# sahaRatul/sela

Hardware: AMD Instinct MI355X
Metric: Msamples/s encode+decode, 16-bit stereo 44.1kHz, 1/2/4/8 GPU; bit-exact vs CPU (higher is better)
Workload: dtype f64+int64

## Files before the change

### sela_amd/csrc/sela_device.h

```cpp
#ifndef SELA_DEVICE_H_
#define SELA_DEVICE_H_

#include <hip/hip_runtime.h>
#include <stdint.h>

#define SELA_TABLE_QUAL static __device__ const
#include "sela_format.h"
#include "sela_hip.h"
#include "sela_hip_debug.h"

namespace sela {

constexpr int kWave = 64;
constexpr int kBlock = SELA_BLOCK;
constexpr int kPerLane = kBlock / kWave;
constexpr int kMaxOrder = SELA_MAX_LPC_ORDER;
constexpr int kCoefWordsCap = 32;
constexpr int kResWordsCap = 2208;
constexpr int kSlotWords = kCoefWordsCap + kResWordsCap;
constexpr int kGroupFrames = 8;

struct BlockMeta {
    uint8_t order;
    uint8_t coef_k;
// ... 134 lines not shown
__device__ __forceinline__ uint32_t zigzag32(int32_t x)
{
    const uint32_t t = (uint32_t)x << 1;
    return x < 0 ? (0u - t - 1u) : t;
}
__device__ __forceinline__ uint32_t words_for_bits(uint64_t bits)
{
    return (uint32_t)ceilf((float)bits / 32.0f);
}

__device__ __forceinline__ double dequant(int i, int32_t q, uint32_t& flags)
{
    int idx = q + 64;
    if (idx < 0 || idx > 127) {
        flags |= SELA_HIP_FLAG_Q_RANGE;
        idx = idx < 0 ? 0 : 127;
    }
    return i == 0 ? SELA_DEQUANT_FIRST[idx] : (i == 1 ? SELA_DEQUANT_SECOND[idx] : SELA_DEQUANT_HIGHER[idx]);
}

__device__ __forceinline__ int64_t q35_trunc(double v, uint32_t& flags)
{
    const double scaled = 34359738368.0 * v;
    if (!(scaled > -9223372036854775808.0 && scaled < 9223372036854775808.0)) {
        flags |= SELA_HIP_FLAG_COEF_OVERFLOW;
        return INT64_MIN;
    }
    return (int64_t)scaled;
}

__device__ __forceinline__ double read_lane(double v, int src_lane )
{
    const uint64_t x = __builtin_bit_cast(uint64_t, v);
    const uint32_t lo = (uint32_t)__builtin_amdgcn_readlane((int)(uint32_t)x, src_lane);
    const uint32_t hi = (uint32_t)__builtin_amdgcn_readlane((int)(uint32_t)(x >> 32), src_lane);
    return __builtin_bit_cast(double, ((uint64_t)hi << 32) | lo);
}
__device__ __forceinline__ double wave_shr1_zero(double v)
{
    const uint64_t x = __builtin_bit_cast(uint64_t, v);
    const uint32_t lo = (uint32_t)__builtin_amdgcn_mov_dpp((int)(uint32_t)x, 0x138 , 0xf, 0xf, true);
    const uint32_t hi = (uint32_t)__builtin_amdgcn_mov_dpp((int)(uint32_t)(x >> 32), 0x138, 0xf, 0xf, true);
    return __builtin_bit_cast(double, ((uint64_t)hi << 32) | lo);
}
__device__ __forceinline__ double wave_shr1(double fill, double v)
{
    const uint64_t f = __builtin_bit_cast(uint64_t, fill), x = __builtin_bit_cast(uint64_t, v);
    const uint32_t lo = (uint32_t)__builtin_amdgcn_update_dpp((int)(uint32_t)f, (int)(uint32_t)x, 0x138 , 0xf, 0xf, false);
    const uint32_t hi = (uint32_t)__builtin_amdgcn_update_dpp((int)(uint32_t)(f >> 32), (int)(uint32_t)(x >> 32), 0x138, 0xf, 0xf, false);
    return __builtin_bit_cast(double, ((uint64_t)hi << 32) | lo);
}

__device__ inline void step_up_regs(double k_lo, double k_hi, int64_t* a, int order, int lane, uint32_t& flags)
{
    double t_lo = lane == 0 ? 1.0 : 0.0, r_lo = lane == 1 ? 1.0 : 0.0;
    double t_hi = 0.0, r_hi = 0.0;
    const int n_lo = order < 62 ? order : 62;
    for (int i = 0; i < n_lo; i++) {
        const double ki = read_lane(k_lo, i);
        const double tn = t_lo + ki * r_lo;
        const double rn = r_lo + ki * t_lo;
        t_lo = tn;
        r_lo = wave_shr1_zero(rn);
    }
    for (int i = 62; i < order; i++) {
        const double ki = i < 64 ? read_lane(k_lo, i) : read_lane(k_hi, i - 64);
        const double tn_lo = t_lo + ki * r_lo, rn_lo = r_lo + ki * t_lo;
        const double tn_hi = t_hi + ki * r_hi, rn_hi = r_hi + ki * t_hi;
        t_lo = tn_lo;
        t_hi = tn_hi;
        const double carry = read_lane(rn_lo, 63);
        r_lo = wave_shr1_zero(rn_lo);
        r_hi = wave_shr1(carry, rn_hi);
    }
    if (lane == 0)
        a[0] = 0;
    else if (lane <= order)
        a[lane] = q35_trunc(-t_lo, flags);
    if (lane + 64 <= order)
        a[lane + 64] = q35_trunc(-t_hi, flags);
    wave_sync();
}

__device__ inline void step_up(const double* kd, int64_t* a, int order, int lane, uint32_t& flags)
{
    const double k_lo = lane < order ? kd[lane] : 0.0;
    const double k_hi = lane + 64 < order ? kd[lane + 64] : 0.0;
    step_up_regs(k_lo, k_hi, a, order, lane, flags);
}

__device__ __forceinline__ void step_up_from_q(uint32_t order, int32_t q_lo, int32_t q_hi, int64_t* a, int lane, uint32_t& flags)
{
    int table_lane = lane;
    asm volatile("" : "+v"(table_lane));
    const double k_lo = (uint32_t)lane < order ? (order <= 1 ? 0.0 : dequant(table_lane, q_lo, flags)) : 0.0;
    const double k_hi = (uint32_t)lane + 64 < order ? dequant(64, q_hi, flags) : 0.0;
    step_up_regs(k_lo, k_hi, a, (int)order, lane, flags);
}

constexpr int kResidencyDecode = 0, kResidencyVerify = 1, kResidencySlots = 2;
uint32_t resident_frames(const void* kernel, int n_waves, size_t lds, int slot = kResidencyDecode);
uint32_t vec_shift_from_for(uint32_t n_frames, int n_waves, uint32_t resident);
int decode_waves(uint32_t channels);

}
#endif
```

### sela_amd/csrc/sela_encode.hip

```cpp
#include <algorithm>
#include <atomic>
#include <random>
#include <vector>

#include "sela_device.h"

namespace sela {

constexpr int kPadC = 64;
constexpr int kHalfEntries = kBlock / 4;
constexpr int kParityLen = kPadC + kHalfEntries + 64;
constexpr int kLastT0 = (kHalfEntries + 64) / 32 - 1;
constexpr int kFirstT1 = (kHalfEntries - kPadC) / 32;
constexpr int kRingHalf = 64;
constexpr int kRingLen = 2 * kRingHalf + 64;
constexpr int kRingsPerXcd = 512;
constexpr int kXcds = 8;
constexpr int kPadS = 128;
constexpr int kSBufWords = (kPadS + kBlock) / 32 * 33;
constexpr int kSmallBase = 8992;
constexpr int kBigBytes = kSmallBase + 3008;
static_assert(kResWordsCap * 4 <= kSmallBase, "packed residue words must fit the dead sample buffer");
static_assert(kSBufWords * 4 <= kSmallBase && kSmallBase % 16 == 0, "sample buffer must end below the analysis arrays");
static_assert(kBigBytes >= 2 * kParityLen * 8, "the FP64 parity arrays must fit");

struct SmallArrays {
    double ac[104];
    double k[104];
    int64_t a[104];
    int32_t q[128];
};
static_assert(sizeof(SmallArrays) + kSmallBase <= kBigBytes, "analysis arrays overflow the LDS plan");

__device__ __forceinline__ void or_bits(uint32_t* buf, uint32_t pos, uint32_t v, uint32_t nbits)
{
    const uint32_t w = pos >> 5, sh = pos & 31;
    atomicOr(&buf[w], v << sh);
    if (sh + nbits > 32)
        atomicOr(&buf[w + 1], v >> (32 - sh));
}

__device__ __forceinline__ void or_bits_both(uint32_t* buf, uint32_t pos, uint32_t v)
{
    const uint64_t wide = (uint64_t)v << (pos & 31);
    uint32_t* const w = buf + (pos >> 5);
    atomicOr(w, (uint32_t)wide);
    atomicOr(w + 1, (uint32_t)(wide >> 32));
}

__device__ __attribute__((noinline)) uint32_t put_long_codeword(uint32_t* buf, uint32_t pos, uint32_t u, uint32_t k);

__device__ __forceinline__ uint32_t put_codeword(uint32_t* buf, uint32_t pos, uint32_t u, uint32_t k)
{
    uint32_t ones = u >> k;
    const uint32_t rem = k ? (__brev(u << (32 - k))) : 0u;
    while (ones >= 32) {
        or_bits(buf, pos, 0xFFFFFFFFu, 32);
        pos += 32;
        ones -= 32;
    }
    if (ones + 1 + k <= 32) {
        or_bits(buf, pos, ((1u << ones) - 1u) | (rem << (ones + 1)), ones + 1 + k);
        return pos + ones + 1 + k;
    }
    or_bits(buf, pos, (1u << ones) - 1u, ones + 1);
    pos += ones + 1;
    if (k) {
        or_bits(buf, pos, rem, k);
        pos += k;
    }
    return pos;
}

__device__ __attribute__((noinline)) uint32_t put_long_codeword(uint32_t* buf, uint32_t pos, uint32_t u, uint32_t k)
{
    return put_codeword(buf, pos, u, k);
}

template <int V>
__device__ __forceinline__ uint64_t rice_shifted_sum(const uint32_t (&u)[V], uint32_t k, bool small, uint32_t& lane_part)
{
    if (small) {
        uint32_t part = 0;
#pragma unroll
        for (int t = 0; t < V; t++)
            part += u[t] >> k;
        asm volatile("" : "+v"(part));
        lane_part = part;
        return wave_sum_small(part);
    }
    uint64_t part = 0;
#pragma unroll
    for (int t = 0; t < V; t++)
        part += u[t] >> k;
    lane_part = (uint32_t)part;
    return wave_sum_40(part);
}

template <int V>
__device__ __forceinline__ void rice_plan(const uint32_t (&u)[V], uint32_t n, uint32_t& best_k, uint64_t& best_bits, uint32_t& lane_or, uint32_t& lane_quotients)
{
    constexpr uint32_t kLast = SELA_MAX_RICE_PARAM - 1;
    lane_or = 0;
#pragma unroll
    for (int t = 0; t < V; t++)
        lane_or |= u[t];
    const bool small = !__any((lane_or >> 20) != 0);
    uint32_t p0, pa, pb, pc;
    const uint64_t t0 = rice_shifted_sum<V>(u, 0, small, p0);
    const uint64_t mean = n ? t0 / n : 0;
    uint32_t k = mean ? 63u - (uint32_t)__clzll(mean) : 0u;
    k = k > kLast - 1 ? kLast - 1 : k;
    uint64_t ta = t0;
    pa = p0;
    if (k)
        ta = rice_shifted_sum<V>(u, k, small, pa);
    uint64_t tb = rice_shifted_sum<V>(u, k + 1, small, pb);
    if (ta - tb <= n) {
        while (k > 0) {
            uint64_t tc = t0;
            pc = p0;
            if (k != 1)
                tc = rice_shifted_sum<V>(u, k - 1, small, pc);
            if (tc - ta > n)
                break;
            k--;
            tb = ta, pb = pa;
            ta = tc, pa = pc;
        }
    } else {
        for (;;) {
            k++;
            ta = tb, pa = pb;
            if (k == kLast)
                break;
            tb = rice_shifted_sum<V>(u, k + 1, small, pb);
            if (ta - tb <= n)
                break;
        }
    }
    best_k = k;
    best_bits = ta + (uint64_t)n * (1 + k);
    lane_quotients = pa;
}

__device__ __forceinline__ double scale_sample(int32_t s)
{
    constexpr double c1 = 0x1.00020004p-15, c2 = 0x1.0002000400080p-60;
    static_assert(c1 == 1.0 / 32768 + 1.0 / (1 << 30) + 1.0 / (1ll << 45) && SELA_SAMPLE_SCALE == 32767.0, "the constants are those of a division by 32767");
    const double x = (double)s;
    const double q = x * c1;
    return __builtin_fma(x, c2, q);
}

template <int kN>
__device__ __forceinline__ void unpack_stereo(uint32_t sig, const uint32_t (&w)[kN], int32_t (&raw)[kN])
{
    if (sig == 0) {
#pragma unroll
        for (int i = 0; i < kN; i++)
            raw[i] = (int32_t)(int16_t)(w[i] & 0xFFFFu);
    } else if (sig == 1) {
#pragma unroll
        for (int i = 0; i < kN; i++)
            raw[i] = (int32_t)w[i] >> 16;
    } else {
#pragma unroll
        for (int i = 0; i < kN; i++)
            raw[i] = (int32_t)(int16_t)(w[i] & 0xFFFFu) - ((int32_t)w[i] >> 16);
    }
}

__device__ __forceinline__ uint32_t stereo_pick(uint32_t sig) { return sig == 0 ? 0x00000001u : sig == 1 ? 0x00010000u : 0xFFFF0001u; }
__device__ __forceinline__ int32_t unpack_stereo_picked(uint32_t pick, uint32_t w)
{
    int32_t s;
    asm("v_dot2_i32_i16 %0, %1, %2, 0" : "=v"(s) : "v"(w), "s"(pick));
    return s;
}

typedef double f64x2 __attribute__((ext_vector_type(2)));
struct MeanFetch {
    f64x2 e0, e1, e2, e3, o0, o1, o2, o3;
};
#define SELA_MEAN_STR2(x) #x
#define SELA_MEAN_STR(x) SELA_MEAN_STR2(x)
#define SELA_MEAN_ISSUE(F, addr, OFF, sum)                                                    \
    asm volatile("ds_read_b128 %0, %9 offset:" #OFF "+0\n\t"                                    \
                 "ds_read_b128 %4, %9 offset:" #OFF "+5120\n\t"                                 \
                 "ds_read_b128 %1, %9 offset:" #OFF "+16\n\t"                                   \
// ... 2163 lines not shown
```

### sela_amd/csrc/sela_encode_tail.inc

```

    SELA_STAMP(5);
#ifndef SELA_TAIL_HAVE_Q
    int order;
    {
        const unsigned long long b_lo = __ballot(fabs(k_lo) > SELA_ORDER_THRESHOLD);
        const unsigned long long b_hi = __ballot(lane < 36 && fabs(k_hi) > SELA_ORDER_THRESHOLD);
        order = b_hi ? 128 - __clzll(b_hi) : (b_lo ? 64 - __clzll(b_lo) : 1);
    }
#endif

    {
#ifndef SELA_TAIL_HAVE_Q
        const double sqrt2 = SELA_SQRT2;
        double v_lo;
        if (lane == 0)
            v_lo = floor(64 * (-1 + (sqrt2 * sqrt(k_lo + 1))));
        else if (lane == 1)
            v_lo = floor(64 * (-1 + (sqrt2 * sqrt(-k_lo + 1))));
        else
            v_lo = floor(64 * k_lo);
        const double v_hi = floor(64 * k_hi);
        const int32_t q_lo = isnan(v_lo) ? 0 : (int32_t)v_lo;
        const int32_t q_hi = isnan(v_hi) ? 0 : (int32_t)v_hi;
#endif
// ... 89 lines not shown
                const int32_t rt = (int32_t)((uint32_t)mine_s[t] - pred_u[t]);
                wide |= (rt >= (1 << 30)) || (rt < -(1 << 30));
            }
        } else {
            double* const c_first = reinterpret_cast<double*>(sm->a);
            double* const c_second = single ? c_first : sm->k;
            for (int j = 1 + lane; j <= order; j += 64) {
                const int64_t aj = sm->a[j];
                const int64_t top = aj >> 20;
                const double lo = (double)(uint32_t)((uint64_t)aj & 0xFFFFFu);
                const double hi = (double)(int32_t)(top >> 16) * 65536.0 + (double)(uint32_t)((uint64_t)top & 0xFFFFu);
                if (single) {
                    c_first[j] = hi * 1048576.0 + lo;
                } else {
                    c_first[j] = lo;
                    c_second[j] = hi;
                }
            }
            wave_sync();
            double win_f[kPerLane], acc_f[kPerLane];
            double half = (double)((int64_t)1 << (SELA_Q_SHIFT - 1));
            asm volatile("" : "+s"(half));
#pragma unroll
            for (int t = 0; t < kPerLane; t++)
                acc_f[t] = half;
            if (single) {
#pragma unroll
                for (int t = 0; t < kPerLane; t++)
                    win_f[t] = (double)mine_s[t];
#pragma unroll 1
                for (int j0 = 0; j0 < order; j0 += 32)
                    fir_taps_f64<0>(j0, order, fir_group_window(sT, lane, j0), fir_group_coefs(c_first, j0), win_f, acc_f);
#pragma unroll
                for (int t = 0; t < kPerLane; t++) {
                    if constexpr (kMode == 4)
                        pred_u[t] = (uint32_t)((int32_t)__builtin_ceil(acc_f[t] * (1.0 / (double)((int64_t)1 << SELA_Q_SHIFT))) - 1);
                    else
                        pred_u[t] = (uint32_t)(int32_t)__builtin_floor(acc_f[t] * (1.0 / (double)((int64_t)1 << SELA_Q_SHIFT)));
                }
            } else {
#pragma unroll 1
                for (int pass = 0; pass < 2; pass++) {
                    const double* const coef = pass ? c_second : c_first;
#pragma unroll
                    for (int t = 0; t < kPerLane; t++)
                        win_f[t] = (double)mine_s[t];
#pragma unroll 1
                    for (int j0 = 0; j0 < order; j0 += 32)
                        fir_taps_f64<0>(j0, order, fir_group_window(sT, lane, j0), fir_group_coefs(coef, j0), win_f, acc_f);
                    const double down = pass ? 1.0 / (double)((int64_t)1 << (SELA_Q_SHIFT - 20)) : 1.0 / 1048576.0;
#pragma unroll
                    for (int t = 0; t < kPerLane; t++) {
                        if constexpr (kMode == 4)
                            acc_f[t] = __builtin_ceil(acc_f[t] * down);
                        else
                            acc_f[t] = __builtin_floor(acc_f[t] * down);
                    }
                }
#pragma unroll
                for (int t = 0; t < kPerLane; t++) {
                    if constexpr (kMode == 4)
                        pred_u[t] = (uint32_t)((int32_t)acc_f[t] - 1);
                    else
                        pred_u[t] = (uint32_t)(int32_t)acc_f[t];
                }
            }
        }
#pragma unroll
        for (int t = 0; t < kPerLane; t++) {
            const int32_t rt = (int32_t)((uint32_t)mine_s[t] - pred_u[t]);
            ru[t] = zigzag32(rt);
#ifdef SELA_TAIL_TRACE_RESIDUES
            if (kTrace && (SELA_TAIL_TRACE_RESIDUES))
                (SELA_TAIL_TRACE_RESIDUES)[(size_t)block_id * kBlock + 32 * lane + t] = rt;
#endif
        }
    }
    wave_sync();

    SELA_STAMP(8);
    uint32_t cu[2];
    cu[0] = 2 * lane < order ? zigzag32(sm->q[2 * lane]) : 0u;
    cu[1] = 2 * lane + 1 < order ? zigzag32(sm->q[2 * lane + 1]) : 0u;
    uint32_t coef_k, coef_or, coef_quotients;
    uint64_t coef_bits;
    rice_plan<2>(cu, (uint32_t)order, coef_k, coef_bits, coef_or, coef_quotients);
    const uint32_t coef_words = words_for_bits(coef_bits);

    if (__any(wide))
        flags |= SELA_HIP_FLAG_RICE_RANGE;
    uint32_t res_k, res_or, res_quotients;
    uint64_t res_bits;
    rice_plan<kPerLane>(ru, (uint32_t)kBlock, res_k, res_bits, res_or, res_quotients);
    uint32_t res_words = words_for_bits(res_bits);
    if (res_words > (uint32_t)kResWordsCap || coef_words > (uint32_t)kCoefWordsCap) {
        flags |= SELA_HIP_FLAG_WORDS_CAP;
        res_words = 0;
    }

    const bool paired = sizes_pub != nullptr && channels == 2 && sig >= 1;
    const uint32_t my_words = coef_words + res_words;
    if (paired && lane == 0)
        store_through(sizes_pub + block_id, sizes_tag | (uint64_t)my_words);

    SELA_STAMP(9);
    if (lane < kCoefWordsCap)
        cw_buf[lane] = 0;
    wave_sync();
    if (!(flags & SELA_HIP_FLAG_WORDS_CAP)) {
        const uint32_t n0 = 2 * lane < order ? (cu[0] >> coef_k) + 1 + coef_k : 0u;
        const uint32_t n1 = 2 * lane + 1 < order ? (cu[1] >> coef_k) + 1 + coef_k : 0u;
        uint32_t pos = wave_exclusive_scan(n0 + n1, lane);
        if (n0)
            pos = put_codeword(cw_buf, pos, cu[0], coef_k);
        if (n1)
            pos = put_codeword(cw_buf, pos, cu[1], coef_k);
    }

    uint64_t other = 0;
    if (paired)
        other = load_through(sizes_pub + (sig == 1 ? block_id + 1 : block_id - 1));

    SELA_STAMP(10);
    uint32_t* const out_words = reinterpret_cast<uint32_t*>(big);
    for (uint32_t w = lane; w < res_words; w += 64)
        out_words[w] = 0;
    const uint32_t lane_bits = res_quotients + (uint32_t)kPerLane * (1 + res_k);
    wave_sync();
    if (res_words) {
        uint32_t pos = wave_exclusive_scan(lane_bits, lane);
#pragma unroll
        for (int t = 0; t < kPerLane; t++) {
            const uint32_t u = ru[t], ones = u >> res_k, len = ones + 1 + res_k;
            if (len <= 32) {
                const uint32_t rem = __builtin_amdgcn_ubfe(__brev(u), 32 - res_k, res_k);
                or_bits_both(out_words, pos, ((1u << ones) - 1u) | (rem << ((ones + 1) & 31)));
                pos += len;
            } else {
                pos = put_long_codeword(out_words, pos, u, res_k);
            }
        }
    }
    wave_sync();

    SELA_STAMP(11);
    uint32_t* slot = slots + (size_t)block_id * kSlotWords;
    bool loser = false;
    if (paired) {
        const uint32_t other_words = (uint32_t)other & 0xFFFu;
        loser = (other & ~(uint64_t)0xFFF) == sizes_tag && (sig == 1 ? other_words < my_words : !(my_words < other_words));
        loser = __builtin_amdgcn_readfirstlane((int)loser) != 0;
    }
    if (loser) {
    } else if (kFused) {
        uint64_t* const slot2 = reinterpret_cast<uint64_t*>(slot);
        if (lane < kCoefWordsCap / 2)
            store_through(slot2 + lane, (uint64_t)cw_buf[2 * lane] | ((uint64_t)cw_buf[2 * lane + 1] << 32));
        const uint64_t* const out2 = reinterpret_cast<const uint64_t*>(out_words);
        for (uint32_t w2 = lane; w2 < (res_words + 1) / 2; w2 += 64)
            store_through(slot2 + kCoefWordsCap / 2 + w2, out2[w2]);
    } else {
        if (lane < (int)coef_words && lane < kCoefWordsCap)
            slot[lane] = cw_buf[lane];
        for (uint32_t w = lane; w < res_words; w += 64)
            slot[kCoefWordsCap + w] = out_words[w];
    }
    const uint32_t all_flags = wave_or(flags);
    if (lane == 0) {
        BlockMeta bm;
        bm.order = (uint8_t)order;
        bm.coef_k = (uint8_t)coef_k;
        bm.res_k = (uint8_t)res_k;
        bm.flags = (uint8_t)(all_flags | form_bits);
        bm.coef_words = (uint16_t)coef_words;
        bm.res_words = (uint16_t)res_words;
        if (kFused)
            store_through(reinterpret_cast<uint64_t*>(meta + block_id), __builtin_bit_cast(uint64_t, bm));
        else
            meta[block_id] = bm;
        if (kTrace) {
            sela_hip_trace* tr = trace + block_id;
            tr->coef_k = coef_k;
            tr->coef_words = coef_words;
            tr->res_k = res_k;
            tr->res_words = res_words;
            tr->flags = all_flags;
        }
    }
```

### sela_amd/csrc/sela_generic.hip

```cpp
#include <hip/hip_runtime.h>

#include <algorithm>
#include <atomic>

#include "sela_device.h"
#include "sela_generic.h"

namespace sela {

hipError_t launch_decode(const uint8_t* d_frames, const uint64_t* d_frame_offsets, uint32_t n_frames, uint32_t channels, int16_t* d_pcm_out, uint32_t* d_status,
    void* d_workspace, hipStream_t stream, hipEvent_t* ev, uint64_t* d_phase_cycles, uint8_t* frame_flags, int recurrence_form, uint32_t synth_priorities,
    const uint32_t* d_n_found, bool zero_status);

namespace {

__device__ __forceinline__ uint64_t wave_sum_wrap(uint64_t v)
{
#pragma unroll
    for (int m = 1; m < 64; m <<= 1) {
        const uint32_t lo = (uint32_t)__shfl_xor((int)(uint32_t)v, m, 64);
        const uint32_t hi = (uint32_t)__shfl_xor((int)(uint32_t)(v >> 32), m, 64);
        v += ((uint64_t)hi << 32) | lo;
    }
    return v;
// ... 367 lines not shown
                        acc_e += pe;
                        acc_o += po;
                    }
                    {
                        const double pe = cj.y * A.y, po = cj.y * A.x;
                        acc_e += pe;
                        acc_o += po;
                    }
                    B = A.y;
                    __builtin_amdgcn_sched_barrier(0);
                }
            } else {
                const int cnt = (int)(n - j0);
                for (int t = 0; t < cnt; t++) {
                    const double cj = read_lane(c_mine, t);
                    const double A = rl[t];
                    const double pe = cj * A, po = cj * B;
                    acc_e += pe;
                    acc_o += po;
                    B = A;
                }
            }
            wave_sync();
        }
    }

    {
        const double ac0 = read_lane(acc_e, 0);
        const double n_e = acc_e / ac0, n_o = acc_o / ac0;
        double g1a = n_o, g1b = wave_shl1(0.0, n_e);
        double g0a = g1a, g0b = g1b;
        double err = 1.0;
        double g = read_lane(g1a, 0);
        double k = -g / err;
        err += g * k;
        if (lane == 0)
            lds.kk[0] = k;
#pragma unroll 1
        for (int i = 1; i < kMaxOrder; i++) {
            const double next = wave_shl1(0.0, g1a);
            const double n1a = g1b + k * g0a, n0a = g1b * k + g0a;
            const double n1b = next + k * g0b, n0b = next * k + g0b;
            g1a = n1a, g0a = n0a, g1b = n1b, g0b = n0b;
            g = read_lane(g1a, 0);
            k = -g / err;
            err += g * k;
            if (lane == 0)
                lds.kk[i] = k;
        }
    }
    wave_sync();
    const double k_lo = lds.kk[lane];
    const double k_hi = lane + 64 < kMaxOrder ? lds.kk[lane + 64] : 0.0;
    wave_sync();

    int order;
    {
        const unsigned long long b_lo = __ballot(fabs(k_lo) > SELA_ORDER_THRESHOLD);
        const unsigned long long b_hi = __ballot(lane + 64 < kMaxOrder && fabs(k_hi) > SELA_ORDER_THRESHOLD);
        order = b_hi ? 128 - __clzll(b_hi) : (b_lo ? 64 - __clzll(b_lo) : 1);
    }
    {
        const double sqrt2 = SELA_SQRT2;
        double v_lo;
        if (lane == 0)
            v_lo = floor(64 * (-1 + (sqrt2 * sqrt(k_lo + 1))));
        else if (lane == 1)
            v_lo = floor(64 * (-1 + (sqrt2 * sqrt(-k_lo + 1))));
        else
            v_lo = floor(64 * k_lo);
        const double v_hi = floor(64 * k_hi);
        const int32_t q_lo = isnan(v_lo) ? 0 : trunc_to_i32(v_lo);
        const int32_t q_hi = isnan(v_hi) ? 0 : trunc_to_i32(v_hi);
        if (lane < order) {
            lds.q[lane] = q_lo;
            lds.kk[lane] = order <= 1 ? 0.0 : dequant(lane, q_lo, flags);
        }
        if (lane + 64 < order) {
            lds.q[lane + 64] = q_hi;
            lds.kk[lane + 64] = dequant(lane + 64, q_hi, flags);
        }
    }
    wave_sync();
    step_up(lds.kk, lds.a, order, lane, flags);
    for (int i = lane; i < kMaxOrder; i += 64)
        q_ws[(size_t)b * kMaxOrder + i] = i < order ? lds.q[i] : 0;

    if ((uint32_t)order >= n)
        flags |= SELA_HIP_FLAG_SHORT_BLOCK;
    bool fp64_taps;
    {
        bool modest = true;
        uint64_t a_abs = 0;
        for (int j = 1 + lane; j <= order; j += 64) {
            const int64_t aj = lds.a[j];
            const uint64_t mag = aj < 0 ? 0 - (uint64_t)aj : (uint64_t)aj;
            modest &= mag < ((uint64_t)1 << 39);
            a_abs += modest ? mag : 0u;
            const int64_t top = aj >> 20;
            lds.af[j] = ((double)(int32_t)(top >> 16) * 65536.0 + (double)(uint32_t)((uint64_t)top & 0xFFFFu)) * 1048576.0 + (double)(uint32_t)((uint64_t)aj & 0xFFFFFu);
        }
        const uint64_t a_sum = wave_sum_wrap(a_abs);
        const uint64_t room = ((uint64_t)1 << 53) - ((uint64_t)1 << (SELA_Q_SHIFT - 1));
        fp64_taps = !__any(!modest) && (a_sum == 0 || (uint64_t)s_mag < room / a_sum) && !force_wrap_taps;
        wave_sync();
    }
    uint64_t t0_lane = 0;
    bool wide = false;
    if (fp64_taps) {
        int32_t* const sT = lds.st;
        for (int m = lane; m < kGenPad; m += 64)
            sT[m + (m >> kGenPadShift)] = 0;
        for (uint32_t i0 = 0; i0 < n; i0 += kGenStretch) {
            if (i0) {
                int32_t keep[2];
#pragma unroll
                for (int h = 0; h < 2; h++) {
                    const int e = kGenStretch + lane + 64 * h;
                    keep[h] = sT[e + (e >> kGenPadShift)];
                }
                wave_sync();
#pragma unroll
                for (int h = 0; h < 2; h++) {
                    const int e = lane + 64 * h;
                    sT[e + (e >> kGenPadShift)] = keep[h];
                }
            }
#pragma unroll 8
            for (int t = 0; t < kGenPerLane; t++) {
                const uint32_t i = i0 + lane + 64 * t;
                const int e = kGenPad + lane + 64 * t;
                sT[e + (e >> kGenPadShift)] = i < n ? s[i] : 0;
            }
            wave_sync();
            const int32_t* mine_s = sT + (kGenPad + kGenPerLane * lane) + ((kGenPad + kGenPerLane * lane) >> kGenPadShift);
            double win_f[kGenPerLane], acc_f[kGenPerLane];
#pragma unroll
            for (int t = 0; t < kGenPerLane; t++) {
                acc_f[t] = (double)((int64_t)1 << (SELA_Q_SHIFT - 1));
                win_f[t] = (double)mine_s[t];
            }
#pragma unroll 1
            for (int j0 = 0; j0 < order; j0 += kGenPerLane)
                gen_taps_f64<0>(j0, order, lane, sT, lds.af, win_f, acc_f);
            int32_t rr[kGenPerLane];
#pragma unroll
            for (int t = 0; t < kGenPerLane; t++) {
                int32_t pred;
                if constexpr (kLossless)
                    pred = (int32_t)__builtin_ceil(acc_f[t] * (1.0 / (double)((int64_t)1 << SELA_Q_SHIFT))) - 1;
                else
                    pred = (int32_t)__builtin_floor(acc_f[t] * (1.0 / (double)((int64_t)1 << SELA_Q_SHIFT)));
                rr[t] = (int32_t)((uint32_t)mine_s[t] - (uint32_t)pred);
            }
            const uint32_t first = i0 + (uint32_t)kGenPerLane * (uint32_t)lane;
#pragma unroll
            for (int t = 0; t < kGenPerLane; t++)
                if (first + t < n) {
                    r[first + t] = rr[t];
                    t0_lane += zigzag32(rr[t]);
                    wide |= (rr[t] >= (1 << 30)) || (rr[t] < -(1 << 30));
                }
            wave_sync();
        }
    } else {
        const uint32_t o = (uint32_t)order;
        int32_t before1 = 0, before2 = 0;
// ... 375 lines not shown

__device__ inline int32_t rice_chunk(RiceScan& sc, const uint8_t* base, uint32_t k, uint32_t count, bool& overrun)
{
    uint64_t my_at = 0;
    uint32_t my_ones = 0;
    for (uint32_t i = 0; i < count; i++) {
        uint64_t at;
        uint32_t ones;
        sc.next(k, at, ones);
        if ((uint32_t)sc.lane == i)
            my_at = at, my_ones = ones;
    }
    const bool live = (uint32_t)sc.lane < count;
    const uint64_t field = my_at + my_ones + 1;
    overrun |= live && field + k > sc.end;
    const uint32_t rem = live ? remainder_bits(base, field, sc.end, k) : 0u;
    const uint32_t u = (my_ones << k) | rem;
    return live ? (int32_t)((u >> 1) ^ (0u - (u & 1u))) : 0;
}

__global__ __launch_bounds__(64) void k_generic_decode(const uint8_t* __restrict__ frames, const uint64_t* __restrict__ frame_offsets, uint64_t base_bytes,
    uint32_t n_frames, uint32_t channels, uint32_t stride, int32_t* __restrict__ dec_ws ,
    GenericSubInfo* __restrict__ info , uint32_t* __restrict__ status,
    const uint32_t* __restrict__ n_frames_found ,
    const uint32_t* __restrict__ left_alone )
{
    __shared__ int64_t a_lds[kMaxOrder + 1];
    __shared__ int32_t q_lds[256];
    const uint32_t sub = blockIdx.x;
    if (sub >= n_frames * channels)
        return;
    if (left_alone && *left_alone == 0)
        return;
    const int lane = threadIdx.x;
    const uint32_t f = sub / channels, c = sub % channels;
    if (n_frames_found && f >= *n_frames_found)
        return;
    const uint8_t* const fb = frames + (frame_offsets[f] - base_bytes);
    const uint64_t fbytes = frame_offsets[f + 1] - frame_offsets[f];
    GenericSubInfo si;
    si.channel = si.type = si.parent = 0, si.n = 0, si.ok = 0;
    uint32_t flags = 0;
    bool ok = fbytes >= 4 && fbytes < (1ull << 31) && fb[0] == 0x00 && fb[1] == 0xFF && fb[2] == 0x55 && fb[3] == 0xAA;
    uint64_t p = 4;
    SelaSubframeHeader h = {};
    for (uint32_t i = 0; ok && i <= c; i++) {
        const uint64_t next = sela_subframe_read_bytes(fb, fbytes, p, &h);
        ok = next != 0;
        if (i < c)
            p = next;
    }
    si.channel = (uint8_t)h.channel, si.type = (uint8_t)h.type, si.parent = (uint8_t)h.parent;
    const uint32_t cw = h.cw, order = h.order, rw = h.rw, n = h.n, ck = h.ck, rk = h.rk;
    ok = ok && sela_subframe_decodable(&h) && n <= stride;
    if (!ok) {
        if (lane == 0) {
            info[sub] = si;
            atomicOr(&status[0], (uint32_t)SELA_HIP_FLAG_BAD_FRAME);
            atomicAdd(&status[1], 1u);
        }
        return;
    }
    si.n = n, si.ok = 1;
    if (n == 0 || n <= order)
        flags |= SELA_HIP_FLAG_SHORT_BLOCK;
    const uint32_t* const fw = reinterpret_cast<const uint32_t*>(fb);
    const uint32_t n_fw = (uint32_t)(fbytes >> 2);
    bool overrun = false;
    RiceScan sc;
    {
        const uint64_t first = 8 * (p + 7);
        sc.start(fw, n_fw, first, first + 32ull * cw, lane);
        for (uint32_t i0 = 0; i0 < order; i0 += 64) {
            const int32_t v = rice_chunk(sc, fb, ck, order - i0 < 64u ? order - i0 : 64u, overrun);
            if (i0 + lane < order)
                q_lds[i0 + lane] = v;
        }
    }
    wave_sync();
    {
        const uint32_t o = order;
        const int32_t q_lo = (uint32_t)lane < o ? q_lds[lane] : 0;
        const int32_t q_hi = (uint32_t)lane + 64 < o ? q_lds[lane + 64] : 0;
        step_up_from_q(o, q_lo, q_hi, a_lds, lane, flags);
    }
    const uint64_t a_lo = (uint32_t)lane + 1 <= order ? (uint64_t)a_lds[lane + 1] : 0;
    const uint64_t a_hi = (uint32_t)lane + 65 <= order ? (uint64_t)a_lds[lane + 65] : 0;
    {
        const uint64_t first = 8 * (p + 12 + 4 * (uint64_t)cw);
        sc.start(fw, n_fw, first, first + 32ull * rw, lane);
    }
    int32_t* const out = dec_ws + (size_t)sub * stride;
    uint64_t p_lo = 0, p_hi = 0;
    for (uint32_t i0 = 0; i0 < n; i0 += 64) {
        const uint32_t cnt = n - i0 < 64u ? n - i0 : 64u;
        const int32_t mine = rice_chunk(sc, fb, rk, cnt, overrun);
        int32_t made = 0;
        for (uint32_t l = 0; l < cnt; l++) {
            const int32_t res = __builtin_amdgcn_readlane(mine, (int)l);
            const uint64_t sum = read_first_lane(p_lo);
            const uint64_t temp = ((uint64_t)1 << (SELA_Q_SHIFT - 1)) - sum;
            const int32_t smp = (int32_t)((uint32_t)res - (uint32_t)(int32_t)((int64_t)temp >> SELA_Q_SHIFT));
            if ((uint32_t)lane == l)
                made = smp;
            if (order > 64) {
                const uint64_t carry = read_first_lane(p_hi);
                const uint32_t nlo = (uint32_t)wave_shl1((int)(uint32_t)carry, (int)(uint32_t)p_lo);
                const uint32_t nhi = (uint32_t)wave_shl1((int)(uint32_t)(carry >> 32), (int)(uint32_t)(p_lo >> 32));
                p_lo = (((uint64_t)nhi << 32) | nlo) + a_lo * (uint64_t)(int64_t)smp;
                p_hi = wave_shl1_zero(p_hi) + a_hi * (uint64_t)(int64_t)smp;
            } else {
                p_lo = wave_shl1_zero(p_lo) + a_lo * (uint64_t)(int64_t)smp;
            }
        }
        if (i0 + lane < n)
            out[i0 + lane] = made;
    }
    if (__any(overrun))
        flags |= SELA_HIP_FLAG_RICE_OVERRUN;
    flags = wave_or(flags);
    if (lane == 0) {
        info[sub] = si;
        if (flags)
            atomicOr(&status[0], flags);
    }
}

constexpr int kCombineThreads = 256;
constexpr uint32_t kCombineSlice = 4096;
template <bool kOut16>
__global__ __launch_bounds__(kCombineThreads) void k_generic_combine(const int32_t* __restrict__ dec_ws, const GenericSubInfo* __restrict__ info, uint32_t n_frames,
    uint32_t channels, uint32_t stride, int32_t* __restrict__ all , uint32_t* __restrict__ counts,
    const uint64_t* __restrict__ sample_offsets, int16_t* __restrict__ pcm_out, uint32_t* __restrict__ status,
    const uint32_t* __restrict__ n_frames_found )
{
    __shared__ uint32_t cnt[256];
    const uint32_t f = blockIdx.x;
    if (f >= n_frames || (n_frames_found && f >= *n_frames_found))
        return;
    const uint32_t t = threadIdx.x;
    const uint32_t lo = blockIdx.y * kCombineSlice, hi = lo + kCombineSlice;
    const bool first_slice = blockIdx.y == 0;
    const GenericSubInfo* const inf = info + (size_t)f * channels;
    int32_t* const fa = all + (size_t)f * channels * stride;
    const int32_t* const fd = dec_ws + (size_t)f * channels * stride;
    for (uint32_t c = t; c < channels; c += kCombineThreads)
        cnt[c] = 0;
    __syncthreads();
    bool bad = false;
    for (uint32_t c = 0; c < channels; c++) {
        const GenericSubInfo si = inf[c];
        if (!si.ok || si.type != 0)
            continue;
        if (si.channel >= channels) {
            bad = true;
            continue;
        }
        const uint32_t end = min(si.n, hi);
        for (uint32_t i = lo + t; i < end; i += kCombineThreads)
            fa[(size_t)si.channel * stride + i] = fd[(size_t)c * stride + i];
        __syncthreads();
        if (t == 0)
            cnt[si.channel] = si.n;
        __syncthreads();
    }
    for (uint32_t c = 0; c < channels; c++) {
        const GenericSubInfo si = inf[c];
// ... 709 lines not shown
```

Baseline: 17490.

## Stream step-up reflection coefficients from LDS with prefetch and add short-codeword fast path

Adds an LDS-based step-up recursion that reads each reflection coefficient as a uniform LDS load, prefetched four stages ahead. This replaces the per-stage cross-lane readlane of the register-resident coefficients and splits out a low-half-only path for orders below 60. The decode path parks the dequantized coefficients in the a[] array before running it, while the generic kernel keeps the old register path. Separately, the residue packer takes a branch-free loop when a wave max shows every codeword fits in 32 bits, using v_bfm for the unary mask. The main risks are the LDS overwrite of a[] during the in-place step-up and a slightly costlier max reduction in place of the OR.

```diff
diff --git a/sela_amd/csrc/sela_device.h b/sela_amd/csrc/sela_device.h
--- a/sela_amd/csrc/sela_device.h
+++ b/sela_amd/csrc/sela_device.h
@@ -240,20 +240,108 @@
     wave_sync();
 }
 
+constexpr int kStepAhead = 4;
+typedef const volatile __attribute__((address_space(3))) uint64_t* LdsStepK;
+__device__ __forceinline__ double step_up_k(LdsStepK kd, int i) { return __builtin_bit_cast(double, (uint64_t)kd[i]); }
+
+template <typename K>
+__device__ inline void step_up_lds(const K* kd_in, int64_t* a, int order, int lane, uint32_t& flags)
+{
+    static_assert(sizeof(K) == 8, "64-bit words");
+    const LdsStepK kd = (LdsStepK)kd_in;
+    double t_lo = lane == 0 ? 1.0 : 0.0, r_lo = lane == 1 ? 1.0 : 0.0;
+    double t_hi = 0.0, r_hi = 0.0;
+    double pf[kStepAhead];
+#pragma unroll
+    for (int u = 0; u < kStepAhead; u++)
+        pf[u] = step_up_k(kd, u);
+    __builtin_amdgcn_s_waitcnt(0xC07F);
+    auto stage_lo = [&](double ki) {
+        const double tn = t_lo + ki * r_lo;
+        const double rn = r_lo + ki * t_lo;
+        t_lo = tn;
+        r_lo = wave_shr1_zero(rn);
+    };
+    auto stage_hi = [&](double ki) {
+        const double tn_lo = t_lo + ki * r_lo, rn_lo = r_lo + ki * t_lo;
+        const double tn_hi = t_hi + ki * r_hi, rn_hi = r_hi + ki * t_hi;
+        t_lo = tn_lo;
+        t_hi = tn_hi;
+        const double carry = read_lane(rn_lo, 63);
+        r_lo = wave_shr1_zero(rn_lo);
+        r_hi = wave_shr1(carry, rn_hi);
+    };
+    static_assert(kStepAhead == 4 && 60 % kStepAhead == 0, "stages 60 .. 63 are one group");
+    const int n_whole = (order < 60 ? order : 60) & ~(kStepAhead - 1);
+    int i = 0;
+    for (; i < n_whole; i += kStepAhead) {
+#pragma unroll
+        for (int u = 0; u < kStepAhead; u++) {
+            stage_lo(pf[u]);
+            pf[u] = step_up_k(kd, i + kStepAhead + u);
+        }
+    }
+    if (order < 60) {
+#pragma unroll
+        for (int u = 0; u < kStepAhead - 1; u++)
+            if (i + u < order)
+                stage_lo(pf[u]);
+    } else {
+#pragma unroll
+        for (int u = 0; u < kStepAhead; u++)
+            if (60 + u < order) {
+                if (u < 2)
+                    stage_lo(pf[u]);
+                else
+                    stage_hi(pf[u]);
+                pf[u] = step_up_k(kd, 64 + u);
+            }
+        for (i = 64; i < order; i += kStepAhead) {
+#pragma unroll
+            for (int u = 0; u < kStepAhead; u++)
+                if (i + u < order) {
+                    stage_hi(pf[u]);
+                    pf[u] = step_up_k(kd, i + kStepAhead + u);
+                }
+        }
+    }
+    if (lane == 0)
+        a[0] = 0;
+    else if (lane <= order)
+        a[lane] = q35_trunc(-t_lo, flags);
+    if (lane + 64 <= order)
+        a[lane + 64] = q35_trunc(-t_hi, flags);
+    wave_sync();
+}
+
+template <bool kFromLds = true>
 __device__ inline void step_up(const double* kd, int64_t* a, int order, int lane, uint32_t& flags)
 {
-    const double k_lo = lane < order ? kd[lane] : 0.0;
-    const double k_hi = lane + 64 < order ? kd[lane + 64] : 0.0;
-    step_up_regs(k_lo, k_hi, a, order, lane, flags);
-}
-
+    if constexpr (kFromLds) {
+        step_up_lds(kd, a, order, lane, flags);
+    } else {
+        const double k_lo = lane < order ? kd[lane] : 0.0;
+        const double k_hi = lane + 64 < order ? kd[lane + 64] : 0.0;
+        step_up_regs(k_lo, k_hi, a, order, lane, flags);
+    }
+}
+
+template <bool kParkInA = true>
 __device__ __forceinline__ void step_up_from_q(uint32_t order, int32_t q_lo, int32_t q_hi, int64_t* a, int lane, uint32_t& flags)
 {
     int table_lane = lane;
     asm volatile("" : "+v"(table_lane));
     const double k_lo = (uint32_t)lane < order ? (order <= 1 ? 0.0 : dequant(table_lane, q_lo, flags)) : 0.0;
     const double k_hi = (uint32_t)lane + 64 < order ? dequant(64, q_hi, flags) : 0.0;
-    step_up_regs(k_lo, k_hi, a, (int)order, lane, flags);
+    if constexpr (kParkInA) {
+        a[lane] = __builtin_bit_cast(int64_t, k_lo);
+        if (lane < kMaxOrder + kStepAhead - 64)
+            a[lane + 64] = __builtin_bit_cast(int64_t, k_hi);
+        wave_sync();
+        step_up_lds(a, a, (int)order, lane, flags);
+    } else {
+        step_up_regs(k_lo, k_hi, a, (int)order, lane, flags);
+    }
 }
 
 constexpr int kResidencyDecode = 0, kResidencyVerify = 1, kResidencySlots = 2;
diff --git a/sela_amd/csrc/sela_encode.hip b/sela_amd/csrc/sela_encode.hip
--- a/sela_amd/csrc/sela_encode.hip
+++ b/sela_amd/csrc/sela_encode.hip
@@ -48,6 +48,13 @@
     atomicOr(w + 1, (uint32_t)(wide >> 32));
 }
 
+__device__ __forceinline__ uint32_t low_ones(uint32_t n)
+{
+    uint32_t m;
+    asm("v_bfm_b32 %0, %1, 0" : "=v"(m) : "v"(n));
+    return m;
+}
+
 __device__ __attribute__((noinline)) uint32_t put_long_codeword(uint32_t* buf, uint32_t pos, uint32_t u, uint32_t k);
 
 __device__ __forceinline__ uint32_t put_codeword(uint32_t* buf, uint32_t pos, uint32_t u, uint32_t k)
@@ -98,14 +105,14 @@
 }
 
 template <int V>
-__device__ __forceinline__ void rice_plan(const uint32_t (&u)[V], uint32_t n, uint32_t& best_k, uint64_t& best_bits, uint32_t& lane_or, uint32_t& lane_quotients)
+__device__ __forceinline__ void rice_plan(const uint32_t (&u)[V], uint32_t n, uint32_t& best_k, uint64_t& best_bits, uint32_t& lane_top, uint32_t& lane_quotients)
 {
     constexpr uint32_t kLast = SELA_MAX_RICE_PARAM - 1;
-    lane_or = 0;
+    lane_top = 0;
 #pragma unroll
     for (int t = 0; t < V; t++)
-        lane_or |= u[t];
-    const bool small = !__any((lane_or >> 20) != 0);
+        lane_top = max(lane_top, u[t]);
+    const bool small = !__any((lane_top >> 20) != 0);
     uint32_t p0, pa, pb, pc;
     const uint64_t t0 = rice_shifted_sum<V>(u, 0, small, p0);
     const uint64_t mean = n ? t0 / n : 0;
diff --git a/sela_amd/csrc/sela_encode_tail.inc b/sela_amd/csrc/sela_encode_tail.inc
--- a/sela_amd/csrc/sela_encode_tail.inc
+++ b/sela_amd/csrc/sela_encode_tail.inc
@@ -195,16 +195,17 @@
     uint32_t cu[2];
     cu[0] = 2 * lane < order ? zigzag32(sm->q[2 * lane]) : 0u;
     cu[1] = 2 * lane + 1 < order ? zigzag32(sm->q[2 * lane + 1]) : 0u;
-    uint32_t coef_k, coef_or, coef_quotients;
+    uint32_t coef_k, coef_top, coef_quotients;
     uint64_t coef_bits;
-    rice_plan<2>(cu, (uint32_t)order, coef_k, coef_bits, coef_or, coef_quotients);
+    rice_plan<2>(cu, (uint32_t)order, coef_k, coef_bits, coef_top, coef_quotients);
     const uint32_t coef_words = words_for_bits(coef_bits);
 
     if (__any(wide))
         flags |= SELA_HIP_FLAG_RICE_RANGE;
-    uint32_t res_k, res_or, res_quotients;
+    uint32_t res_k, res_top, res_quotients;
     uint64_t res_bits;
-    rice_plan<kPerLane>(ru, (uint32_t)kBlock, res_k, res_bits, res_or, res_quotients);
+    rice_plan<kPerLane>(ru, (uint32_t)kBlock, res_k, res_bits, res_top, res_quotients);
+    const bool res_all_short = (wave_max_u32(res_top) >> res_k) + 1 + res_k <= 32;
     uint32_t res_words = words_for_bits(res_bits);
     if (res_words > (uint32_t)kResWordsCap || coef_words > (uint32_t)kCoefWordsCap) {
         flags |= SELA_HIP_FLAG_WORDS_CAP;
@@ -242,15 +243,29 @@
     wave_sync();
     if (res_words) {
         uint32_t pos = wave_exclusive_scan(lane_bits, lane);
-#pragma unroll
-        for (int t = 0; t < kPerLane; t++) {
-            const uint32_t u = ru[t], ones = u >> res_k, len = ones + 1 + res_k;
-            if (len <= 32) {
-                const uint32_t rem = __builtin_amdgcn_ubfe(__brev(u), 32 - res_k, res_k);
-                or_bits_both(out_words, pos, ((1u << ones) - 1u) | (rem << ((ones + 1) & 31)));
-                pos += len;
-            } else {
-                pos = put_long_codeword(out_words, pos, u, res_k);
+        if (res_all_short) {
+            uint32_t k_v = res_k, rem_at = 32 - res_k;
+            asm volatile("" : "+v"(k_v));
+            asm volatile("" : "+s"(rem_at));
+#pragma unroll
+            for (int t = 0; t < kPerLane; t++) {
+                const uint32_t u = ru[t], ones = u >> res_k;
+                const uint32_t rem = __builtin_amdgcn_ubfe(__brev(u), rem_at, k_v);
+                const uint32_t next = ones + 1;
+                or_bits_both(out_words, pos, low_ones(ones) | (rem << (next & 31)));
+                pos = pos + next + k_v;
+            }
+        } else {
+#pragma unroll
+            for (int t = 0; t < kPerLane; t++) {
+                const uint32_t u = ru[t], ones = u >> res_k, len = ones + 1 + res_k;
+                if (len <= 32) {
+                    const uint32_t rem = __builtin_amdgcn_ubfe(__brev(u), 32 - res_k, res_k);
+                    or_bits_both(out_words, pos, ((1u << ones) - 1u) | (rem << ((ones + 1) & 31)));
+                    pos += len;
+                } else {
+                    pos = put_long_codeword(out_words, pos, u, res_k);
+                }
             }
         }
     }
diff --git a/sela_amd/csrc/sela_generic.hip b/sela_amd/csrc/sela_generic.hip
--- a/sela_amd/csrc/sela_generic.hip
+++ b/sela_amd/csrc/sela_generic.hip
@@ -473,7 +473,7 @@
         }
     }
     wave_sync();
-    step_up(lds.kk, lds.a, order, lane, flags);
+    step_up<false>(lds.kk, lds.a, order, lane, flags);
     for (int i = lane; i < kMaxOrder; i += 64)
         q_ws[(size_t)b * kMaxOrder + i] = i < order ? lds.q[i] : 0;
 
@@ -1015,7 +1015,7 @@
         const uint32_t o = order;
         const int32_t q_lo = (uint32_t)lane < o ? q_lds[lane] : 0;
         const int32_t q_hi = (uint32_t)lane + 64 < o ? q_lds[lane + 64] : 0;
-        step_up_from_q(o, q_lo, q_hi, a_lds, lane, flags);
+        step_up_from_q<false>(o, q_lo, q_hi, a_lds, lane, flags);
     }
     const uint64_t a_lo = (uint32_t)lane + 1 <= order ? (uint64_t)a_lds[lane + 1] : 0;
     const uint64_t a_hi = (uint32_t)lane + 65 <= order ? (uint64_t)a_lds[lane + 65] : 0;
```

After: 17740 (median of 6 runs). 1.4% higher.
